# Asherchi/Stereo_Match_Traditional

Measured on AMD Instinct MI355X. Metric: Mdisparities/s (HxWxD/s) + ms/pair, AD-Census 1920x1080 D=192, higher is better.
Workload: dtype f32; 1 GPU; AD-Census 9x7 both views + WTA, 1920x1080 D=192 (adcensus_1080p_d192); parallelism=pairs sharded over 1 GPU(s), backend=none (single process), ranks_joined=1, ranks_joined_how=all_reduce(SUM) of 1 per rank over the job's communicator, world_size=1, launcher=none

## Files before the change

### stereo_match_traditional_amd/csrc/adcensus.hip

```cpp
#include "smt_common.h"
#include "adcensus_internal.h"
#include <math.h>
#include <stdlib.h>
#include <string.h>
#include <algorithm>
#include <new>
#include <type_traits>

namespace {

constexpr int TJ = 64;
constexpr int NT = 256;

struct Tables {
    uint64_t *cenA[2];
    uint64_t *cenX[2];
    uint64_t *mask;
    uint8_t *u8[2];
    float *lut;
    uint16_t *rank;
    int *flag;
    int WX;
    int edge_col;
    unsigned long long *stamp;
// ... 296 lines not shown
    }
}

#ifndef SMT_SHARED_KNOCKOUT
#define SMT_SHARED_KNOCKOUT 0
#endif
constexpr int SH_RING = 512;
constexpr int SH_RING_N = SH_RING + 4;
constexpr unsigned long long SH_NOKEY = ~0ull;
__host__ __device__ inline int shared_id_hi(int W, int D) { return W - 3 - D; }
__host__ __device__ inline int shared_pub_hi(int W) { return W - 4; }
__host__ __device__ inline bool shared_in_set(int c, int hi) { return (unsigned)(c - 3) <= (unsigned)(hi - 3) && hi >= 3; }
__host__ __device__ inline bool shared_publishes(int j, int c, int W, int pubhi) { return j <= W - 4 && shared_in_set(c, pubhi); }
__host__ __device__ inline unsigned long long shared_key(unsigned cost_bits, int d) { return ((unsigned long long)cost_bits << 32) | (unsigned)d; }
__host__ __device__ inline int shared_ring_base(int t, int C) { return (int)((unsigned)(t - (C - 1)) & (unsigned)(SH_RING - 1)); }
constexpr int SH_SPILL = SH_RING_N - SH_RING;
__host__ __device__ constexpr bool shared_walk_groups(int C, int Dfull) { return C == 3 && Dfull == 192; }
__host__ __device__ constexpr bool shared_ring_grouped(int C, int Dfull) { return C == 3 && Dfull == 192; }
static_assert(!shared_ring_grouped(3, 192) || shared_walk_groups(3, 192), "");
__host__ __device__ inline int shared_ring_slot(int t0, int u, int k, int C) { return shared_ring_base(t0, C) + u + (C - 1 - k); }
__host__ __device__ constexpr int shared_ring_spill(int C, bool grouped) { return grouped ? 2 * (C - 1) : C - 1; }
static_assert(shared_ring_spill(3, true) <= SH_SPILL && shared_ring_spill(4, false) <= SH_SPILL, "");
constexpr int SH_RUN = 4;
__host__ __device__ inline int shared_wg_chunks(int nbx, int H, int K, long b, int &i, int &bx)
{
    const long nb = (long)nbx * H, per = (nb + 7) >> 3, cl = (b >> 3) * K;
    if (cl >= per) return 0;
    const long c = (b & 7) * per + cl;
    if (c >= nb) return 0;
    i = (int)(c / nbx);
    bx = (int)(c - (long)i * nbx);
    long n = per - cl < nb - c ? per - cl : nb - c;
    return (int)(n < K ? n : K);
}
__host__ __device__ inline int shared_run_len(int nbx, int bx, int left)
{
    const int n = nbx - bx < SH_RUN ? nbx - bx : SH_RUN;
    return n < left ? n : left;
}
__host__ __device__ inline void shared_run_flush_range(int S, int E, int D, int pubhi, int &lo, int &hi)
{
    lo = S - D + 1 < 3 ? 3 : S - D + 1; hi = E > pubhi ? pubhi : E;
}
__host__ __device__ inline bool shared_complete(int c, int S, int E, int D) { return c >= S && c + D - 1 <= E; }
__host__ __device__ inline bool shared_complete(int c, int S, int E, int D, int idhi) { return c <= idhi && shared_complete(c, S, E, D); }
__host__ __device__ inline void shared_edge_range(int c, int W, int D, int &lo, int &hi)
{
    lo = c >= 3 && W - 3 - c > 0 ? W - 3 - c : 0;
    hi = W + 3 - c < D - 1 ? W + 3 - c : D - 1;
}
constexpr int SH_CONV_PX = 16 * 256;
constexpr int SH_EDGE_PX = 4 * 256;
constexpr int SH_EDGE0_PX = 16 * 4;
__host__ __device__ inline int shared_conv_items(int H, int W) { return (int)(((long)H * W + SH_CONV_PX - 1) / SH_CONV_PX); }
__host__ __device__ inline int shared_edge_cols(int W, int D) { return W - 1 - shared_id_hi(W, D); }
__host__ __device__ inline int shared_edge_col_items(int H, int W, int D)
// ... 213 lines not shown
                        const unsigned long long b = __ballot(ml == m);
                        const int first = __builtin_ctzll(b);
                        int kk = C - 1;
#pragma unroll
                        for (int k = C - 2; k >= 0; k--)
                            if ((unsigned)__builtin_amdgcn_readlane((int)key[k], first) == m) kk = k;
                        const int wd = first * C + kk;
                        res = (lane == q) ? wd : res;
                    }
                    const int ns = (VIEW == 0) ? (u + 1) % C : u % C;
                    rc[ns] = nc; rv[ns] = nv;
                }
            }
            anc_a += 16u * C; val_a += 2u * C;
            nx_a += 8u * C; nv_a += 2u * C;
        }
    };
    if (interior) run(std::false_type{});
    else run(std::true_type{});
    const int jw = j0 + p0 + lane;
    if (disp && lane < npx) disp[(size_t)i * W + jw] = (float)res;
}

__host__ __device__ inline bool chunk_decode(int nbx, int H, int nviews, int K, long b, int t, int &view, int &i, int &bx)
{
    const long nb = (long)nbx * H * nviews;
    const long per = (nb + 7) >> 3;
    const long cl = (b >> 3) * K + t;
    if (cl >= per) return false;
    const long c = (b & 7) * per + cl;
    if (c >= nb) return false;
    const long rows = (long)nbx * H;
    view = (int)(c / rows);
    const long r = c - (long)view * rows;
    i = (int)(r / nbx);
    bx = (int)(r - (long)i * nbx);
    return true;
}
__host__ __device__ inline int maps_groups(int nbx, int H, int nviews, int K)
{
    const long per = ((long)nbx * H * nviews + 7) >> 3;
    return (int)(8 * ((per + K - 1) / K));
}
__device__ __forceinline__ bool chunk_of_block(int nbx, int H, int nviews, int &view, int &i, int &bx, long b = -1)
{
    const long nb = (long)nbx * H * nviews;
    const long per = (nb + 7) >> 3;
    if (b < 0) b = blockIdx.x;
    const long c = (b & 7) * per + (b >> 3);
    if (c >= nb) return false;
    const long rows = (long)nbx * H;
    view = (int)(c / rows);
    const long r = c - (long)view * rows;
    i = (int)(r / nbx);
    bx = (int)(r - (long)i * nbx);
    return true;
}

template <int C, int VIEW, bool FULL>
__global__ void __launch_bounds__(NT) k_cost_fast(int H, int W, int D, Tables T, float *__restrict__ vol,
                                                  float *__restrict__ disp, int nbx)
{
    int view, i, bx;
    if (!chunk_of_block(nbx, H, 1, view, i, bx)) return;
    cost_fast_body<C, VIEW, FULL>(H, W, D, T, vol, disp, i, bx);
}

template <int C, bool FULL, bool NTS = true>
__global__ void __launch_bounds__(NT) k_cost_fast2(int H, int W, int D, Tables T, float *__restrict__ vol0,
                                                   float *__restrict__ vol1, float *__restrict__ disp0,
                                                   float *__restrict__ disp1, int nbx)
{
    int view, i, bx;
    if (!chunk_of_block(nbx, H, 2, view, i, bx)) return;
    unsigned long long t0 = 0, r0 = 0;
    if (T.stamp) { t0 = __builtin_amdgcn_s_memtime(); r0 = __builtin_amdgcn_s_memrealtime(); }
    if (view == 0) cost_fast_body<C, 0, FULL, NTS>(H, W, D, T, vol0, disp0, i, bx);
    else cost_fast_body<C, 1, FULL, NTS>(H, W, D, T, vol1, disp1, i, bx);
    if (T.stamp && threadIdx.x == 0) {
        unsigned long long *s = T.stamp + 4 * (size_t)blockIdx.x;
        s[0] = t0; s[1] = r0; s[2] = __builtin_amdgcn_s_memtime(); s[3] = __builtin_amdgcn_s_memrealtime();
    }
}

struct FusedGrid { int cgroups, pgroups, every, slots, groups; };
__host__ __device__ inline FusedGrid fused_grid(int ncost, int nprep)
{
    FusedGrid f;
    f.cgroups = ncost >> 3;
    f.pgroups = (nprep + 7) >> 3;
    f.every = f.cgroups / (f.pgroups > 0 ? f.pgroups : 1);
    if (f.every < 1) f.every = 1;
    f.slots = f.cgroups / f.every;
    f.groups = f.cgroups + (f.pgroups > f.slots ? f.pgroups : f.slots);
    return f;
}
__host__ __device__ inline bool fused_decode(const FusedGrid &f, int g, int &idx)
{
    const int period = f.every + 1, inter = f.slots * period;
    if (g < inter) {
        const int q = g / period, r = g - q * period;
        if (r == f.every) { idx = q; return true; }
        idx = q * f.every + r;
        return false;
    }
    const int g2 = g - inter, crest = f.cgroups - f.slots * f.every;
    if (g2 < crest) { idx = f.slots * f.every + g2; return false; }
    idx = f.slots + (g2 - crest);
    return true;
}

template <int C, bool FULL, bool NTS = true>
__global__ void __launch_bounds__(NT, 8) k_cost_fast2p(int H, int W, int D, Tables T, float *__restrict__ vol0,
// ... 57 lines not shown
            va = T.u8[view][(size_t)i * W + j];
        }
    }
    template <unsigned VSCALE, int TABN, int NBUF>
    __device__ __forceinline__ void store(MapsLds<C, TABN, NBUF> &ml, int buf, int Drt) const
    {
        const int D = FULL ? 64 * C : Drt, NX = FTJ + D, tid = threadIdx.x;
#pragma unroll
        for (int n = 0; n < NE; n++) {
            const int e = tid - (FULL ? 0 : XPAD) + n * NT;
            if (e < NX + (FULL ? 0 : XPAD)) {
                ml.st[buf].cenx[XPAD + e] = cen[n];
                ml.st[buf].valx[XPAD + e] = (uint16_t)(VSCALE * val[n]);
            }
        }
        if (tid < FTJ) { ml.st[buf].anc[tid] = anc; ml.st[buf].vala[tid] = (uint16_t)(VSCALE * va); }
    }
};

template <int C, bool FULL, int MODE>
__global__ void __launch_bounds__(NT) k_cost_maps2p(int H, int W, int D, Tables T, float *__restrict__ disp0,
                                                    float *__restrict__ disp1, int nbx, int K, int ncost, int nprep,
                                                    const float *__restrict__ nL, const float *__restrict__ nR,
                                                    Tables Tn, int ptx)
{
    static_assert(PNT == NT, "");
    constexpr int TABN = MapsCfg<MODE>::TABN, NBUF = MapsCfg<MODE>::NBUF;
    static_assert(2 * PSR * PSW * 4 <= TABN * 2 && 320 * 4 <= TABN * 2, "");
    __shared__ MapsLds<C, TABN, NBUF> lds;
    uint16_t *s_tab = lds.tab;
    long b = blockIdx.x;
    if (nprep > 0) {
        const FusedGrid f = fused_grid(ncost, nprep);
        int idx;
        const bool table = fused_decode(f, (int)(blockIdx.x >> 3), idx);
        b = idx * 8 + (int)(blockIdx.x & 7);
        if (table) {
            uint32_t (*sw)[PSW] = (uint32_t (*)[PSW])s_tab;
            if (b < nprep) prep_tile(nL, nR, H, W, Tn, (int)b % ptx, (int)b / ptx, ptx, sw, sw + PSR);
            return;
        }
    }
    const int tid = threadIdx.x;
    if (MODE == MODE_MAPS_RANK) {
        typedef unsigned u32x4 __attribute__((ext_vector_type(4)));
        for (int e = tid; e < RANK_N / 8; e += NT) ((u32x4 *)s_tab)[e] = ((const u32x4 *)T.rank)[e];
    } else {
        for (int e = tid; e < 320; e += NT) ((float *)s_tab)[e] = T.lut[e];
    }
    auto next = [&](int t, int &view, int &i, int &bx) {
        for (; t < K; t++) {
            if (!chunk_decode(nbx, H, 2, K, b, t, view, i, bx)) return K;
            if (view == 0 ? disp0 : disp1) return t;
        }
        return K;
    };
    MapsStage<C, FULL> st;
    int view = 0, i = 0, bx = 0;
    int t = next(0, view, i, bx);
    if (t < K) st.load(view, i, bx, W, D, T);
    bool first = true;
    int buf = 0;
    while (t < K) {
        if (NBUF == 1 && !first) __syncthreads();
        first = false;
        st.template store<MODE == MODE_MAPS_RANK ? 64u : 4u>(lds, buf, D);
        __syncthreads();
        const int cv = view, ci = i, cbx = bx;
        t = next(t + 1, view, i, bx);
        if (t < K) st.load(view, i, bx, W, D, T);
        if (cv == 0) cost_fast_body<C, 0, FULL, true, MODE>(H, W, D, T, nullptr, disp0, ci, cbx, &lds, buf);
        else cost_fast_body<C, 1, FULL, true, MODE>(H, W, D, T, nullptr, disp1, ci, cbx, &lds, buf);
        buf = NBUF == 1 ? 0 : buf ^ 1;
    }
}
// ... 276 lines not shown
        if (!shared_edge0_px(item - ncol, it, (int)(threadIdx.x >> 6), H, i, c)) return;
        const size_t p = (size_t)i * W + c;
        const uint64_t acen = T.cenA[1][p], amask = T.mask[p];
        const int va = T.u8[1][p];
        int lo, hi;
        shared_edge_range(c, W, D, lo, hi);
        unsigned long long k = SH_NOKEY;
        for (int d = lo + lane; d <= hi; d += 64) k = min(k, shared_edge_key(T, i, W, acen, amask, va, c + d, d));
#pragma unroll
        for (int s = 32; s >= 1; s >>= 1) k = min(k, (unsigned long long)__shfl_xor((long long)k, s));
        if (lane == 0) dispR[p] = (float)(unsigned)k;
    }
}

#ifndef SMT_SHARED_MIN_WAVES
#define SMT_SHARED_MIN_WAVES 7
#endif
template <int C, bool FULL>
__global__ void __launch_bounds__(NT, SMT_SHARED_MIN_WAVES) k_cost_maps_shared(int H, int W, int D, Tables T, float *__restrict__ disp0,
                                                         float *__restrict__ disp1, unsigned long long *__restrict__ keys,
                                                         int nbx, int K, int pubhi, int ncost, int nprep,
                                                         const float *__restrict__ nL, const float *__restrict__ nR,
                                                         Tables Tn, int ptx, int nconv, int nedge,
                                                         unsigned long long *__restrict__ ckeys, float *__restrict__ cdisp)
{
    static_assert(PNT == NT && NT == 256, "");
    static_assert(2 * PSR * PSW * 4 <= PREP_LDS_U16 * 2 && 320 * 4 <= PREP_LDS_U16 * 2, "");
    __shared__ RunLds<C> lds;
    __shared__ unsigned long long ring[SH_RING_N];
    long b;
    {
        const FusedGrid f = fused_grid(ncost, nprep + nconv + nedge);
        int idx;
        const bool table = fused_decode(f, (int)(blockIdx.x >> 3), idx);
        b = idx * 8 + (int)(blockIdx.x & 7);
        if (table) {
            int item;
            const int kind = shared_aux_decode((int)b, nprep, nconv, nedge, item);
            if (kind == AUX_PREP) {
                uint32_t (*sw)[PSW] = (uint32_t (*)[PSW])lds.tab;
                prep_tile(nL, nR, H, W, Tn, item % ptx, item / ptx, ptx, sw, sw + PSR);
            } else if (kind == AUX_CONV) shared_conv_item(ckeys, cdisp, (long)H * W, item);
            else if (kind == AUX_EDGE) shared_edge_item(T, H, W, FULL ? 64 * C : D, disp1, keys, item);
            return;
        }
    }
    const int tid = threadIdx.x;
    int i = 0, bx = 0;
    int left = shared_wg_chunks(nbx, H, K, b, i, bx);
    if (left == 0) return;
    for (int e = tid; e < 320; e += NT) ((float *)lds.tab)[e] = T.lut[e];
    const int Dd = FULL ? 64 * C : D;
    const int idhi = shared_id_hi(W, Dd);
    for (int e = tid; e < SH_RING_N; e += NT) ring[e] = SH_NOKEY;
    RunStage<C, FULL> st;
    int n = shared_run_len(nbx, bx, left);
    st.load(i, FTJ * bx, n, W, D, T);
    for (;;) {
        st.store(lds, n, D);
        __syncthreads();
        const int ci = i, cS = FTJ * bx, cn = n;
        left -= n; bx += n;
        if (bx == nbx) { bx = 0; i++; }
        n = shared_run_len(nbx, bx, left);
        shared_run_walk<C, FULL>(H, W, D, disp0, ci, cS, cn, &lds, ring, pubhi);
        if (n > 0) st.load(i, FTJ * bx, n, W, D, T);
        __syncthreads();
        const int cE = cS + FTJ * cn - 1;
        int lo, hi;
        shared_run_flush_range(cS, cE, Dd, pubhi, lo, hi);
        shared_flush<C, shared_ring_grouped(C, FULL ? 64 * C : 0)>(ring, ci, W, Dd, lo, hi, cS, cE, idhi, disp1, keys);
        if (n <= 0) break;
// ... 64 lines not shown
    hipStream_t stream;
    float *vol[2];
    Tables T;
    Tables TS[2];
    hipStream_t prep_stream;
    hipEvent_t in_ready, prep_done[2], cost_done[2];
    long n_pairs;
    hipEvent_t *ev;
    bool timing;
    bool force_generic;
    long n_timed;
    long n_seen;
    int timing_stride;
    bool *ev_merged;
    bool plain_stores;
    float store_mode_ms[2];
    int place_tries;
    float place_ms;
    unsigned long long *skeys[2];
    bool conv_pending;
    int conv_map;
    float *conv_dR;
    bool vol_lent, vol_pending;
};

SMT_API const char *smt_strerror(int s)
{
    switch (s) {
    case SMT_OK: return "ok";
    case SMT_ERR_ARG: return "invalid argument";
    case SMT_ERR_HIP: return "HIP runtime error";
    case SMT_ERR_ALLOC: return "device allocation failed";
    case SMT_ERR_DOMAIN: return "image values outside the integer 0..255 domain";
    case SMT_ERR_REF_UB: return "reference behaviour undefined for these inputs";
    case SMT_ERR_STATE: return "call order violated";
    default: return "unknown status";
    }
}
SMT_API int smt_version(void) { return SMT_VERSION; }
SMT_API int smt_last_hip_error(void) { return g_smt_last_hip; }
SMT_API int smt_device_count(int *n)
{
    if (!n) return SMT_ERR_ARG;
    SMT_HIP(hipGetDeviceCount(n));
    return SMT_OK;
}
// ... 169 lines not shown
            memcpy(&bits, &f, 4);
            kv[a * 64 + c] = ((uint64_t)bits << 32) | (uint32_t)(a * 64 + c);
        }
    std::sort(kv, kv + RANK_N);
    int r = -1;
    uint32_t prev = 0;
    for (int n = 0; n < RANK_N; n++) {
        const uint32_t bits = (uint32_t)(kv[n] >> 32);
        if (n == 0 || bits != prev) r++;
        prev = bits;
        rank[(uint32_t)kv[n]] = (uint16_t)r;
    }
    delete[] kv;
    return true;
}

static void flush_conversion(smt_adcensus *h)
{
    if (!h->conv_pending) return;
    const long N = (long)h->H * h->W;
    hipLaunchKernelGGL(k_shared_convert, dim3((unsigned)shared_conv_items(h->H, h->W)), dim3(NT), 0, h->stream,
                       h->skeys[h->conv_map], h->conv_dR, N);
    h->conv_pending = false;
}

static int adcensus_create(int H, int W, int D, float sigmaC, float sigmaS, unsigned flags, smt_adcensus **out)
{
    if (!out || H <= 0 || W <= 0 || D <= 0 || D > SMT_MAX_DISPARITY || !(sigmaC > 0.0f) || !(sigmaS > 0.0f) ||
        (long long)H * W >= (1ll << 31))
        return SMT_ERR_ARG;
    smt_adcensus *h = new (std::nothrow) smt_adcensus();
    if (!h) return SMT_ERR_ALLOC;
    h->device = smt_current_device();
    h->H = H; h->W = W; h->D = D; h->sigmaC = sigmaC; h->sigmaS = sigmaS;
    h->stream = nullptr; h->timing = false; h->force_generic = false; h->ev = nullptr; h->n_timed = 0; h->n_seen = 0; h->timing_stride = 1; h->ev_merged = nullptr;
    h->n_pairs = 0;
    const size_t N = (size_t)H * W, V = N * D;
    const int WX = W + 4;
    int rc = place_volumes(h, !(flags & SMT_ADCENSUS_NO_PLACEMENT_SEARCH));
    auto alloc = [&](void **p, size_t bytes) { if (rc == SMT_OK) rc = smt_malloc(p, bytes); };
    alloc((void **)&h->TS[0].lut, 320 * 4);
    alloc((void **)&h->TS[0].rank, RANK_N * 2);
    alloc((void **)&h->TS[0].flag, 4);
    for (int t = 0; t < 2; t++) {
        h->TS[t].WX = WX;
        h->TS[t].stamp = nullptr;
// ... 15 lines not shown
        smt_adcensus_destroy(h);
        return SMT_ERR_HIP;
    }
    for (int t = 0; t < 2; t++)
        if (hipEventCreateWithFlags(&h->prep_done[t], hipEventDisableTiming) != hipSuccess ||
            hipEventCreateWithFlags(&h->cost_done[t], hipEventDisableTiming) != hipSuccess) {
            smt_adcensus_destroy(h);
            return SMT_ERR_HIP;
        }
    float lut[320];
    build_lut(sigmaC, sigmaS, lut);
    uint16_t *rank = new (std::nothrow) uint16_t[RANK_N];
    if (!rank || !build_rank(lut, rank)) { delete[] rank; smt_adcensus_destroy(h); return SMT_ERR_ALLOC; }
    const bool rank_ok = hipMemcpy(h->TS[0].rank, rank, RANK_N * 2, hipMemcpyHostToDevice) == hipSuccess;
    delete[] rank;
    if (!rank_ok || hipMemcpy(h->TS[0].lut, lut, sizeof(lut), hipMemcpyHostToDevice) != hipSuccess ||
        hipMemset(h->vol[0], 0, V * 4) != hipSuccess || hipMemset(h->vol[1], 0, V * 4) != hipSuccess ||
        hipMemset(h->TS[0].flag, 0, 4) != hipSuccess || hipMemset(h->skeys[0], 0xFF, N * 8) != hipSuccess ||
        hipMemset(h->skeys[1], 0xFF, N * 8) != hipSuccess) {
        smt_adcensus_destroy(h);
        return SMT_ERR_HIP;
    }
    calibrate_store_mode(h, !(flags & SMT_ADCENSUS_NO_STORE_CALIBRATION));
    *out = h;
    return SMT_OK;
}

SMT_API int smt_adcensus_create(int H, int W, int D, float sigmaC, float sigmaS, smt_adcensus **out)
{
    return adcensus_create(H, W, D, sigmaC, sigmaS, 0u, out);
}

SMT_API int smt_adcensus_create_ex(int device, int H, int W, int D, float sigmaC, float sigmaS, unsigned flags, smt_adcensus **out)
{
    if (flags & ~(unsigned)(SMT_ADCENSUS_NO_PLACEMENT_SEARCH | SMT_ADCENSUS_NO_STORE_CALIBRATION)) return SMT_ERR_ARG;
    if (device < 0) return adcensus_create(H, W, D, sigmaC, sigmaS, flags, out);
    int n = 0;
    if (hipGetDeviceCount(&n) != hipSuccess || device >= n) return SMT_ERR_ARG;
    smt_dev_guard dev_guard(device);
    return adcensus_create(H, W, D, sigmaC, sigmaS, flags, out);
}

SMT_API int smt_adcensus_create_on(int device, int H, int W, int D, float sigmaC, float sigmaS, smt_adcensus **out)
{
    int n = 0;
    if (hipGetDeviceCount(&n) != hipSuccess || device < 0 || device >= n) return SMT_ERR_ARG;
// ... 45 lines not shown
    h->T.edge_col = h->TS[0].edge_col = h->TS[1].edge_col = col;
    return SMT_OK;
}

template <int C, bool FULL>
static void launch_cost(smt_adcensus *h, int view0, int nviews, float *d0, float *d1)
{
    const int D = h->D;
    dim3 grid((h->W + TJ - 1) / TJ, h->H, nviews);
    const int NX = TJ + D;
    size_t shm = (size_t)NX * 8 + TJ * 16 + 320 * 4 + NX + TJ;
    shm = (shm + 15) & ~(size_t)15;
    hipLaunchKernelGGL((k_cost<C, FULL>), grid, dim3(NT), shm, h->stream, h->H, h->W, D, h->T,
                       view0, h->vol[0], h->vol[1], d0, d1);
}

static int maps_chunks()
{
    const char *env = getenv("SMT_MAPS_CHUNKS");
    const int k = env ? atoi(env) : 0;
    return k >= 1 && k <= 64 ? k : 4;
}

static bool maps_shared()
{
    const char *env = getenv("SMT_MAPS_SHARED");
    return !(env && env[0] == '0' && env[1] == 0);
}
static bool maps_shared_shape(int W, int D)
{
    if (shared_id_hi(W, D) < 3) return false;
    const char *env = getenv("SMT_MAPS_SHARED");
    return D <= 192 || (env && env[0] == 'f');
}

static bool shared_finish_apart()
{
    const char *env = getenv("SMT_SHARED_FINISH");
    return env && strcmp(env, "apart") == 0;
}

static bool pair_takes_shared(const smt_adcensus *h, int views, const float *dL, const float *dR, bool maps)
{
    if (!(views == SMT_VIEW_BOTH && maps) || h->force_generic || (h->D + 63) / 64 > 4) return false;
    const char *env = getenv("SMT_MAPS_KERNEL");
    return !(env && env[0] == 'r') && dL && dR && maps_shared_shape(h->W, h->D) && maps_shared();
}

static int prep_items(int H, int W, int &ptx)
{
    ptx = (W + PTW - 1) / PTW;
    const int pty = (H + PTH - 1) / PTH, eb = (H + PNT / 16 - 1) / (PNT / 16);
    return ptx * (pty + (eb + ptx - 1) / ptx);
}

template <int C, bool FULL>
static void launch_fast(smt_adcensus *h, int views, float *dL, float *dR, const float *nL, const float *nR, bool maps)
{
    const int nbx = (h->W + FTJ - 1) / FTJ;
    auto blocks = [&](int nviews) { return dim3((unsigned)(((long)nbx * h->H * nviews + 7) / 8 * 8)); };
    if (views == SMT_VIEW_BOTH && maps) {
        const int K = maps_chunks();
        const int ncost = maps_groups(nbx, h->H, 2, K);
        int nprep = 0, ptx = 1;
        unsigned grid = (unsigned)ncost;
        if (nL) {
            nprep = prep_items(h->H, h->W, ptx);
            grid = 8u * (unsigned)fused_grid(ncost, nprep).groups;
        }
        const Tables &Tn = h->TS[(h->n_pairs + 1) & 1];
        const char *env = getenv("SMT_MAPS_KERNEL");
        if (pair_takes_shared(h, views, dL, dR, maps)) {
            const int km = (int)(h->n_pairs & 1);
            if (h->conv_pending && h->conv_map == km) flush_conversion(h);
            const bool carried = h->conv_pending;
            const int ncs = maps_groups(nbx, h->H, 1, K), Dd = FULL ? 64 * C : h->D;
            const int nconv = carried ? shared_conv_items(h->H, h->W) : 0, nedge = shared_edge_items(h->H, h->W, Dd);
            const unsigned gs = 8u * (unsigned)fused_grid(ncs, nprep + nconv + nedge).groups;
            hipLaunchKernelGGL((k_cost_maps_shared<C, FULL>), dim3(gs), dim3(NT), 0, h->stream, h->H, h->W, h->D, h->T, dL, dR,
                               h->skeys[km], nbx, K, shared_pub_hi(h->W), ncs, nprep, nL, nR, Tn, ptx, nconv, nedge,
                               carried ? h->skeys[h->conv_map] : nullptr, carried ? h->conv_dR : nullptr);
            if (SMT_SHARED_KNOCKOUT != 2) { h->conv_pending = true; h->conv_map = km; h->conv_dR = dR; }
            else h->conv_pending = false;
            if (shared_finish_apart()) flush_conversion(h);
            return;
        }
        if (env && env[0] == 'r')
            hipLaunchKernelGGL((k_cost_maps2p<C, FULL, MODE_MAPS_RANK>), dim3(grid), dim3(NT), 0, h->stream, h->H, h->W,
                               h->D, h->T, dL, dR, nbx, K, ncost, nprep, nL, nR, Tn, ptx);
        else
            hipLaunchKernelGGL((k_cost_maps2p<C, FULL, MODE_MAPS_FLOAT>), dim3(grid), dim3(NT), 0, h->stream, h->H, h->W,
                               h->D, h->T, dL, dR, nbx, K, ncost, nprep, nL, nR, Tn, ptx);
        return;
    }
    if (views == SMT_VIEW_BOTH && nL) {
        const int ncost = (int)blocks(2).x;
        const int ptx = (h->W + PTW - 1) / PTW, pty = (h->H + PTH - 1) / PTH;
        const int eb = (h->H + PNT / 16 - 1) / (PNT / 16);
        const int nprep = ptx * (pty + (eb + ptx - 1) / ptx);
        const unsigned grid = 8u * (unsigned)fused_grid(ncost, nprep).groups;
        const Tables &Tn = h->TS[(h->n_pairs + 1) & 1];
        if (h->plain_stores)
            hipLaunchKernelGGL((k_cost_fast2p<C, FULL, false>), dim3(grid), dim3(NT), 0, h->stream, h->H, h->W, h->D, h->T,
                               h->vol[0], h->vol[1], dL, dR, nbx, ncost, nprep, nL, nR, Tn, ptx);
        else
            hipLaunchKernelGGL((k_cost_fast2p<C, FULL, true>), dim3(grid), dim3(NT), 0, h->stream, h->H, h->W, h->D, h->T,
                               h->vol[0], h->vol[1], dL, dR, nbx, ncost, nprep, nL, nR, Tn, ptx);
        return;
    }
    if (views == SMT_VIEW_BOTH) {
        if (h->plain_stores)
            hipLaunchKernelGGL((k_cost_fast2<C, FULL, false>), blocks(2), dim3(NT), 0, h->stream, h->H, h->W, h->D, h->T, h->vol[0],
                               h->vol[1], dL, dR, nbx);
        else
            hipLaunchKernelGGL((k_cost_fast2<C, FULL, true>), blocks(2), dim3(NT), 0, h->stream, h->H, h->W, h->D, h->T, h->vol[0],
// ... 235 lines not shown
    const int pubhi = shared_pub_hi(W);
    const bool grouped = shared_ring_grouped(C, D == 64 * C ? D : 0);
    const size_t N = (size_t)H * W;
    static const float pal[] = {0.0f, 0.0f, 0.25f, 0.25f, 1.5f, 0.7265625f, 0.7265625f, 1.9999999f, 0.25f, 1e-30f};
    auto hash_bits = [&](int i, int j, int d, unsigned salt) {
        uint32_t x = (uint32_t)i * 0x9E3779B1u ^ (uint32_t)j * 0x85EBCA77u ^ (uint32_t)d * 0xC2B2AE3Du ^ seed * 0x27D4EB2Fu ^ salt;
        x ^= x >> 15; x *= 0x2C1B3C6Du; x ^= x >> 12; x *= 0x297A2D39u; x ^= x >> 15;
        float f = seed % 3 == 1 ? 0.5f : (seed % 3 == 2 && (x & 3)) ? (float)(x >> 12) * (1.0f / 1048576.0f) : pal[(x >> 4) % 10];
        uint32_t bits;
        memcpy(&bits, &f, 4);
        return bits;
    };
    auto cost_bits = [&](int i, int j, int d) { return hash_bits(i, j, d, 0u); };
    auto right_bits = [&](int i, int c, int d) {
        if (c >= 3 && c + d <= W - 4) return cost_bits(i, c + d, d);
        return hash_bits(i, c, std::min(d, W + 3 - c), 0x5BD1E995u);
    };
    unsigned long long *keys = new (std::nothrow) unsigned long long[N];
    unsigned *val = new (std::nothrow) unsigned[N]();
    unsigned char *nw = new (std::nothrow) unsigned char[N]();
    int rc = (keys && val && nw) ? SMT_OK : SMT_ERR_ALLOC;
    for (size_t p = 0; rc == SMT_OK && p < N; p++) keys[p] = SH_NOKEY;
    if (rc == SMT_OK && idhi >= 3) {
        const int nleft = maps_groups(nbx, H, 1, K);
        unsigned long long ring[SH_RING_N];
        int owner[SH_RING_N];
        for (long b = 0; b < nleft && rc == SMT_OK; b++) {
            for (int e = 0; e < SH_RING_N; e++) ring[e] = SH_NOKEY;
            int view, i, bx, ni, nbxn;
            int left = shared_wg_chunks(nbx, H, K, b, i, bx);
            for (int t = 0; t < K; t++)
                if (chunk_decode(nbx, H, 1, K, b, t, view, ni, nbxn) != (t < left)) rc = SMT_ERR_STATE;
            for (int t = 0; left > 0 && rc == SMT_OK;) {
                const int n = shared_run_len(nbx, bx, left);
                if (n < 1 || n > SH_RUN) { rc = SMT_ERR_STATE; break; }
                for (int u = 0; u < n; u++)
                    if (!chunk_decode(nbx, H, 1, K, b, t + u, view, ni, nbxn) || ni != i || nbxn != bx + u) rc = SMT_ERR_STATE;
                const int S = 64 * bx, E = S + 64 * n - 1;
                for (int e = 0; e < SH_RING_N; e++) owner[e] = -1;
                for (int j = S; j <= E && j < W; j++)
                    for (int lane = 0; lane < 64; lane++)
                        for (int k = 0; k < C; k++) {
                            const int dl = lane * C, d = dl + k, tcol = j - dl;
                            if (d >= D || !shared_publishes(j, tcol - k, W, pubhi)) continue;
                            const int u = grouped ? ((j - S) % (FPW * n)) % C : 0;
                            const int s = shared_ring_slot(tcol - u, u, k, C);
                            if (s < 0 || s >= SH_RING_N) { rc = SMT_ERR_STATE; continue; }
                            if (owner[s] != -1 && owner[s] != tcol - k) rc = SMT_ERR_STATE;
                            owner[s] = tcol - k;
                            ring[s] = std::min(ring[s], shared_key(cost_bits(i, j, d), d));
                        }
                int lo, hi;
                shared_run_flush_range(S, E, D, pubhi, lo, hi);
                for (int c = lo; c <= hi; c++) {
                    const int s = c & (SH_RING - 1);
                    unsigned long long k = ring[s];
                    ring[s] = SH_NOKEY;
                    if (s < shared_ring_spill(C, grouped)) { k = std::min(k, ring[SH_RING + s]); ring[SH_RING + s] = SH_NOKEY; }
                    const size_t p = (size_t)i * W + c;
                    if (shared_complete(c, S, E, D, idhi)) {
// ... 77 lines not shown
        for (size_t p = 0; p < N && rc == SMT_OK; p++)
            if (val2[p] != val[p] || nw2[p] != nw[p] || keys2[p] != keys[p]) rc = SMT_ERR_STATE;
        delete[] keys2; delete[] val2; delete[] nw2;
    }
    for (int i = 0; i < H && rc == SMT_OK; i++)
        for (int c = 0; c < W && rc == SMT_OK; c++) {
            const size_t p = (size_t)i * W + c;
            if (idhi < 3) { if (nw[p]) rc = SMT_ERR_STATE; continue; }
            if (keys[p] != SH_NOKEY) rc = SMT_ERR_STATE;
            float mn = 0.0f;
            int want = 0;
            for (int d = 0; d < D; d++) {
                const uint32_t bits = right_bits(i, c, d);
                float f;
                memcpy(&f, &bits, 4);
                if (d == 0 || f < mn) { mn = f; want = d; }
            }
            if (nw[p] != 1 || val[p] != (unsigned)want) rc = SMT_ERR_STATE;
        }
    delete[] keys; delete[] val; delete[] nw;
    return rc;
}

SMT_API int smt_adcensus_selftest_shared_aux_grid(int ncost, int nprep, int nedge, int nconv)
{
    if (ncost <= 0 || (ncost & 7) || nprep < 0 || nedge < 0 || nconv < 0) return SMT_ERR_ARG;
    const int naux = nprep + nconv + nedge;
    const FusedGrid f = fused_grid(ncost, naux);
    if (8L * f.groups < (long)ncost + naux) return SMT_ERR_STATE;
    unsigned char *cost = new (std::nothrow) unsigned char[(size_t)ncost]();
    unsigned char *aux = new (std::nothrow) unsigned char[(size_t)naux + 1]();
    int rc = (cost && aux) ? SMT_OK : SMT_ERR_ALLOC;
    for (long blk = 0; blk < 8L * f.groups && rc == SMT_OK; blk++) {
        int idx = -1;
        const bool table = fused_decode(f, (int)(blk >> 3), idx);
        if (idx < 0) { rc = SMT_ERR_STATE; break; }
        const long b = (long)idx * 8 + (blk & 7);
        if (!table) {
            if (b >= ncost || cost[b]++) rc = SMT_ERR_STATE;
            continue;
        }
        int item = -1;
        const int kind = shared_aux_decode((int)b, nprep, nconv, nedge, item);
        if (kind == AUX_NONE) { if (b < naux) rc = SMT_ERR_STATE; continue; }
        const int n = kind == AUX_PREP ? nprep : kind == AUX_CONV ? nconv : nedge;
        const int base = kind == AUX_PREP ? 0 : kind == AUX_CONV ? nprep : nprep + nconv;
        if (item < 0 || item >= n || base + item != b || aux[b]++) rc = SMT_ERR_STATE;
    }
    for (int c = 0; c < ncost && rc == SMT_OK; c++) if (cost[c] != 1) rc = SMT_ERR_STATE;
    for (int a = 0; a < naux && rc == SMT_OK; a++) if (aux[a] != 1) rc = SMT_ERR_STATE;
    delete[] cost; delete[] aux;
    return rc;
}

SMT_API int smt_adcensus_selftest_shared_aux(int H, int W, int D, int K, int first, int last)
{
    if (H <= 0 || W <= 0 || D <= 0 || D > 256 || K < 1 || K > 64 || (long)H * W > (1L << 24)) return SMT_ERR_ARG;
    const int idhi = shared_id_hi(W, D), nbx = (W + FTJ - 1) / FTJ;
    if (idhi < 3) return SMT_ERR_ARG;
    int ptx;
    const int ncost = maps_groups(nbx, H, 1, K), nprep = last ? 0 : prep_items(H, W, ptx);
    const int nconv = first ? 0 : shared_conv_items(H, W), nedge = shared_edge_items(H, W, D);
    int rc = smt_adcensus_selftest_shared_aux_grid(ncost, nprep, nedge, nconv);
    if (rc != SMT_OK) return rc;
    const long N = (long)H * W;
    unsigned char *seen = new (std::nothrow) unsigned char[(size_t)N]();
    if (!seen) return SMT_ERR_ALLOC;
    for (int item = 0; item < shared_conv_items(H, W); item++)
        for (int it = 0; it < SH_CONV_PX / 512; it++)
            for (int tid = 0; tid < 256; tid++) {
                long p;
                long p0;
                (void)shared_conv_px(item, 0, tid, N, p0);
                const bool in = shared_conv_px(item, it, tid, N, p);
                if (p != p0 + 512L * it) rc = SMT_ERR_STATE;
                if (!in) continue;
                if (p < 0 || (p & 1)) { rc = SMT_ERR_STATE; continue; }
                for (long e = p; e < p + 2 && e < N; e++) if (seen[e]++) rc = SMT_ERR_STATE;
            }
    for (long p = 0; p < N; p++) { if (seen[p] != 1) rc = SMT_ERR_STATE; seen[p] = 0; }
    const int ncol = shared_edge_col_items(H, W, D);
    for (int item = 0; item < nedge; item++)
        for (int it = 0; it < (item < ncol ? SH_EDGE_PX / 256 : SH_EDGE0_PX / 4); it++)
            for (int t = 0; t < (item < ncol ? 256 : 4); t++) {
                int i = -1, c = -1;
                if (!(item < ncol ? shared_edge_px(item, it, t, H, W, D, i, c) : shared_edge0_px(item - ncol, it, t, H, i, c)))
                    continue;
                const bool in = i >= 0 && i < H && (item < ncol ? c > idhi && c < W : c >= 0 && c < 3);
                if (!in || seen[(long)i * W + c]++) rc = SMT_ERR_STATE;
            }
    for (int i = 0; i < H; i++)
        for (int c = 0; c < W; c++) {
            const bool edge = c < 3 || c > idhi;
            if (seen[(long)i * W + c] != (edge ? 1 : 0)) rc = SMT_ERR_STATE;
            int lo, hi;
            shared_edge_range(c, W, D, lo, hi);
            if (c > idhi && c <= W - 4 && (lo > hi || lo < 1 || c + lo != W - 3)) rc = SMT_ERR_STATE;
            if (edge && (lo < 0 || hi > D - 1 || lo > hi)) rc = SMT_ERR_STATE;
        }
    delete[] seen;
    return rc;
}

SMT_API int smt_adcensus_selftest_cost_rank(float sigmaC, float sigmaS)
{
    if (!(sigmaC > 0.0f) || !(sigmaS > 0.0f)) return SMT_ERR_ARG;
    float lut[320];
    build_lut(sigmaC, sigmaS, lut);
    uint16_t *rank = new (std::nothrow) uint16_t[RANK_N];
    float *sum = new (std::nothrow) float[RANK_N];
    float *uniq = new (std::nothrow) float[RANK_N];
    int rc = (rank && sum && uniq && build_rank(lut, rank)) ? SMT_OK : SMT_ERR_ALLOC;
    int nu = 0;
    if (rc == SMT_OK) {
        for (int e = 0; e < RANK_N; e++) {
            sum[e] = lut[e >> 6] + lut[256 + (e & 63)];
            uint32_t bits;
            memcpy(&bits, &sum[e], 4);
            if (!(sum[e] >= 0.0f && sum[e] < INFINITY) || (bits >> 31)) rc = SMT_ERR_STATE;
            uniq[e] = sum[e];
        }
        std::sort(uniq, uniq + RANK_N);
        nu = (int)(std::unique(uniq, uniq + RANK_N) - uniq);
    }
    for (int e = 0; e < RANK_N && rc == SMT_OK; e++) {
        const int below = (int)(std::lower_bound(uniq, uniq + nu, sum[e]) - uniq);
// ... 180 lines not shown
```

### stereo_match_traditional_amd/csrc/adcensus_internal.h

```cpp
#pragma once
#include "smt_common.h"

int adcensus_batch_pairs(smt_adcensus *h, const float *L, const float *R, int n, int views, float *dispL,
                         float *dispR, int sched, bool prepped, const float *nL, const float *nR, bool maps_ok,
                         bool last_volumes);
bool adcensus_fused_both_views(const smt_adcensus *h);
SMT_API int smt_adcensus_selftest_shared_keys(int H, int W, int D, int K, unsigned seed);
SMT_API int smt_adcensus_selftest_shared_aux_grid(int ncost, int nprep, int nedge, int nconv);
SMT_API int smt_adcensus_selftest_shared_aux(int H, int W, int D, int K, int first, int last);
```

Baseline: 1.984 million Mdisp/s.

## Taper chunk spans at grid tail to balance the maps kernel's last wave

Workgroups normally process K chunks each. This change lets the final groups take half-K or single-chunk spans, so the tail of the grid finishes more evenly. The tail sizes come from occupancy-derived resident-block counts that are queried at create time. By default n1 is set to one resident wave of single-chunk groups whenever the grid exceeds one wave. Fused aux/prep groups are interleaved only inside the body, so tail groups hold pure cost work. The cost is more groups with per-group table-load overhead and more decode logic.

After: 2.029 million Mdisp/s (median of 6 runs). 1.02x the previous value.

```diff
diff --git a/stereo_match_traditional_amd/csrc/adcensus.hip b/stereo_match_traditional_amd/csrc/adcensus.hip
--- a/stereo_match_traditional_amd/csrc/adcensus.hip
+++ b/stereo_match_traditional_amd/csrc/adcensus.hip
@@ -342,16 +342,49 @@
 __host__ __device__ constexpr int shared_ring_spill(int C, bool grouped) { return grouped ? 2 * (C - 1) : C - 1; }
 static_assert(shared_ring_spill(3, true) <= SH_SPILL && shared_ring_spill(4, false) <= SH_SPILL, "");
 constexpr int SH_RUN = 4;
-__host__ __device__ inline int shared_wg_chunks(int nbx, int H, int K, long b, int &i, int &bx)
-{
-    const long nb = (long)nbx * H, per = (nb + 7) >> 3, cl = (b >> 3) * K;
-    if (cl >= per) return 0;
+__host__ __device__ inline long maps_span_tails(long per, int K, int &n2, int &n1)
+{
+    const int K2 = K > 1 ? K >> 1 : 1;
+    if (n1 < 0) n1 = 0;
+    if (n2 < 0) n2 = 0;
+    if (n1 > per) n1 = (int)per;
+    const long rem = per - n1;
+    if ((long)n2 * K2 > rem) n2 = (int)(rem / K2);
+    return rem - (long)n2 * K2;
+}
+__host__ __device__ inline int maps_span(long per, int K, int n2, int n1, long g, long &first)
+{
+    const long body = maps_span_tails(per, K, n2, n1);
+    first = g * K;
+    if (first < body) return (int)(body - first < K ? body - first : K);
+    const int K2 = K > 1 ? K >> 1 : 1;
+    const long gt = g - (body + K - 1) / K;
+    if (gt < n2) { first = body + gt * K2; return K2; }
+    first = body + (long)n2 * K2 + (gt - n2);
+    return gt - n2 < n1 ? 1 : 0;
+}
+__host__ __device__ inline long maps_span_body(long per, int K, int n2, int n1)
+{
+    return (maps_span_tails(per, K, n2, n1) + K - 1) / K;
+}
+__host__ __device__ inline long maps_span_groups(long per, int K, int n2, int n1)
+{
+    const long nbody = maps_span_body(per, K, n2, n1);
+    (void)maps_span_tails(per, K, n2, n1);
+    return nbody + n2 + n1;
+}
+__host__ __device__ inline int shared_wg_chunks(int nbx, int H, int K, long b, int &i, int &bx, int n2 = 0, int n1 = 0)
+{
+    const long nb = (long)nbx * H, per = (nb + 7) >> 3;
+    long cl;
+    const int m = maps_span(per, K, n2, n1, b >> 3, cl);
+    if (m <= 0) return 0;
     const long c = (b & 7) * per + cl;
     if (c >= nb) return 0;
     i = (int)(c / nbx);
     bx = (int)(c - (long)i * nbx);
-    long n = per - cl < nb - c ? per - cl : nb - c;
-    return (int)(n < K ? n : K);
+    const long n = nb - c;
+    return (int)(n < m ? n : m);
 }
 __host__ __device__ inline int shared_run_len(int nbx, int bx, int left)
 {
@@ -611,12 +644,10 @@
     if (disp && lane < npx) disp[(size_t)i * W + jw] = (float)res;
 }
 
-__host__ __device__ inline bool chunk_decode(int nbx, int H, int nviews, int K, long b, int t, int &view, int &i, int &bx)
+__host__ __device__ inline bool chunk_at(int nbx, int H, int nviews, long b, long cl, int &view, int &i, int &bx)
 {
     const long nb = (long)nbx * H * nviews;
     const long per = (nb + 7) >> 3;
-    const long cl = (b >> 3) * K + t;
-    if (cl >= per) return false;
     const long c = (b & 7) * per + cl;
     if (c >= nb) return false;
     const long rows = (long)nbx * H;
@@ -626,10 +657,24 @@
     bx = (int)(r - (long)i * nbx);
     return true;
 }
-__host__ __device__ inline int maps_groups(int nbx, int H, int nviews, int K)
+__host__ __device__ inline bool chunk_decode(int nbx, int H, int nviews, int K, long b, int t, int &view, int &i, int &bx,
+                                             int n2 = 0, int n1 = 0)
 {
     const long per = ((long)nbx * H * nviews + 7) >> 3;
-    return (int)(8 * ((per + K - 1) / K));
+    long first;
+    if (t >= maps_span(per, K, n2, n1, b >> 3, first)) return false;
+    return chunk_at(nbx, H, nviews, b, first + t, view, i, bx);
+}
+__host__ __device__ inline int maps_groups(int nbx, int H, int nviews, int K, int n2 = 0, int n1 = 0)
+{
+    const long per = ((long)nbx * H * nviews + 7) >> 3;
+    return (int)(8 * maps_span_groups(per, K, n2, n1));
+}
+__host__ __device__ inline int maps_body_groups(int nbx, int H, int nviews, int K, int n2, int n1)
+{
+    const long per = ((long)nbx * H * nviews + 7) >> 3;
+    (void)maps_span_tails(per, K, n2, n1);
+    return n2 + n1 > 0 ? (int)maps_span_body(per, K, n2, n1) : 0;
 }
 __device__ __forceinline__ bool chunk_of_block(int nbx, int H, int nviews, int &view, int &i, int &bx, long b = -1)
 {
@@ -673,11 +718,17 @@
 }
 
 struct FusedGrid { int cgroups, pgroups, every, slots, groups; };
-__host__ __device__ inline FusedGrid fused_grid(int ncost, int nprep)
+__host__ __device__ inline FusedGrid fused_grid(int ncost, int nprep, int cbody = 0)
 {
     FusedGrid f;
     f.cgroups = ncost >> 3;
     f.pgroups = (nprep + 7) >> 3;
+    if (cbody > 0 && f.pgroups > 0 && cbody >= f.pgroups && cbody < f.cgroups) {
+        f.every = cbody / f.pgroups;
+        f.slots = f.pgroups;
+        f.groups = f.cgroups + f.pgroups;
+        return f;
+    }
     f.every = f.cgroups / (f.pgroups > 0 ? f.pgroups : 1);
     if (f.every < 1) f.every = 1;
     f.slots = f.cgroups / f.every;
@@ -781,7 +832,7 @@
 __global__ void __launch_bounds__(NT) k_cost_maps2p(int H, int W, int D, Tables T, float *__restrict__ disp0,
                                                     float *__restrict__ disp1, int nbx, int K, int ncost, int nprep,
                                                     const float *__restrict__ nL, const float *__restrict__ nR,
-                                                    Tables Tn, int ptx)
+                                                    Tables Tn, int ptx, int n2, int n1, int cbody)
 {
     static_assert(PNT == NT, "");
     constexpr int TABN = MapsCfg<MODE>::TABN, NBUF = MapsCfg<MODE>::NBUF;
@@ -790,7 +841,7 @@
     uint16_t *s_tab = lds.tab;
     long b = blockIdx.x;
     if (nprep > 0) {
-        const FusedGrid f = fused_grid(ncost, nprep);
+        const FusedGrid f = fused_grid(ncost, nprep, cbody);
         int idx;
         const bool table = fused_decode(f, (int)(blockIdx.x >> 3), idx);
         b = idx * 8 + (int)(blockIdx.x & 7);
@@ -807,9 +858,11 @@
     } else {
         for (int e = tid; e < 320; e += NT) ((float *)s_tab)[e] = T.lut[e];
     }
+    long c0;
+    const int m = maps_span((((long)nbx * H * 2) + 7) >> 3, K, n2, n1, b >> 3, c0);
     auto next = [&](int t, int &view, int &i, int &bx) {
-        for (; t < K; t++) {
-            if (!chunk_decode(nbx, H, 2, K, b, t, view, i, bx)) return K;
+        for (; t < m; t++) {
+            if (!chunk_at(nbx, H, 2, b, c0 + t, view, i, bx)) return K;
             if (view == 0 ? disp0 : disp1) return t;
         }
         return K;
@@ -1132,7 +1185,8 @@
                                                          int nbx, int K, int pubhi, int ncost, int nprep,
                                                          const float *__restrict__ nL, const float *__restrict__ nR,
                                                          Tables Tn, int ptx, int nconv, int nedge,
-                                                         unsigned long long *__restrict__ ckeys, float *__restrict__ cdisp)
+                                                         unsigned long long *__restrict__ ckeys, float *__restrict__ cdisp,
+                                                         int n2, int n1, int cbody)
 {
     static_assert(PNT == NT && NT == 256, "");
     static_assert(2 * PSR * PSW * 4 <= PREP_LDS_U16 * 2 && 320 * 4 <= PREP_LDS_U16 * 2, "");
@@ -1140,7 +1194,7 @@
     __shared__ unsigned long long ring[SH_RING_N];
     long b;
     {
-        const FusedGrid f = fused_grid(ncost, nprep + nconv + nedge);
+        const FusedGrid f = fused_grid(ncost, nprep + nconv + nedge, cbody);
         int idx;
         const bool table = fused_decode(f, (int)(blockIdx.x >> 3), idx);
         b = idx * 8 + (int)(blockIdx.x & 7);
@@ -1157,7 +1211,7 @@
     }
     const int tid = threadIdx.x;
     int i = 0, bx = 0;
-    int left = shared_wg_chunks(nbx, H, K, b, i, bx);
+    int left = shared_wg_chunks(nbx, H, K, b, i, bx, n2, n1);
     if (left == 0) return;
     for (int e = tid; e < 320; e += NT) ((float *)lds.tab)[e] = T.lut[e];
     const int Dd = FULL ? 64 * C : D;
@@ -1268,6 +1322,7 @@
     int conv_map;
     float *conv_dR;
     bool vol_lent, vol_pending;
+    int maps_resident[3];
 };
 
 SMT_API const char *smt_strerror(int s)
@@ -1483,6 +1538,34 @@
     hipLaunchKernelGGL(k_shared_convert, dim3((unsigned)shared_conv_items(h->H, h->W)), dim3(NT), 0, h->stream,
                        h->skeys[h->conv_map], h->conv_dR, N);
     h->conv_pending = false;
+}
+
+template <int C, bool FULL>
+static void query_maps_resident(smt_adcensus *h, int cus)
+{
+    int n[3] = {0, 0, 0};
+    if (hipOccupancyMaxActiveBlocksPerMultiprocessor(&n[0], k_cost_maps_shared<C, FULL>, NT, 0) != hipSuccess) n[0] = 0;
+    if (hipOccupancyMaxActiveBlocksPerMultiprocessor(&n[1], k_cost_maps2p<C, FULL, MODE_MAPS_FLOAT>, NT, 0) != hipSuccess) n[1] = 0;
+    if (hipOccupancyMaxActiveBlocksPerMultiprocessor(&n[2], k_cost_maps2p<C, FULL, MODE_MAPS_RANK>, NT, 0) != hipSuccess) n[2] = 0;
+    for (int t = 0; t < 3; t++) h->maps_resident[t] = n[t] > 0 ? cus / 8 * n[t] : 0;
+}
+static void set_maps_resident(smt_adcensus *h)
+{
+    h->maps_resident[0] = h->maps_resident[1] = h->maps_resident[2] = 0;
+    int cus = 0;
+    if (hipDeviceGetAttribute(&cus, hipDeviceAttributeMultiprocessorCount, h->device) != hipSuccess || cus < 8) return;
+    switch ((h->D + 63) / 64 * 2 + (h->D % 64 == 0 ? 1 : 0)) {
+    case 3: query_maps_resident<1, true>(h, cus); break;
+    case 5: query_maps_resident<2, true>(h, cus); break;
+    case 7: query_maps_resident<3, true>(h, cus); break;
+    case 9: query_maps_resident<4, true>(h, cus); break;
+    case 2: query_maps_resident<1, false>(h, cus); break;
+    case 4: query_maps_resident<2, false>(h, cus); break;
+    case 6: query_maps_resident<3, false>(h, cus); break;
+    case 8: query_maps_resident<4, false>(h, cus); break;
+    default: break;
+    }
+    (void)hipGetLastError();
 }
 
 static int adcensus_create(int H, int W, int D, float sigmaC, float sigmaS, unsigned flags, smt_adcensus **out)
@@ -1544,6 +1627,7 @@
         return SMT_ERR_HIP;
     }
     calibrate_store_mode(h, !(flags & SMT_ADCENSUS_NO_STORE_CALIBRATION));
+    set_maps_resident(h);
     *out = h;
     return SMT_OK;
 }
@@ -1635,6 +1719,21 @@
     return k >= 1 && k <= 64 ? k : 4;
 }
 
+constexpr int TAPER_N2_HALVES = 0, TAPER_N1_HALVES = 2;
+static void maps_taper(int S, long per, int K, int &n2, int &n1)
+{
+    n2 = n1 = 0;
+    const char *env = getenv("SMT_MAPS_TAPER");
+    if (env && env[0]) {
+        int a = 0, b = 0;
+        if (sscanf(env, "%d,%d", &a, &b) == 2 && a >= 0 && b >= 0) { n2 = a; n1 = b; }
+    } else if (S > 0 && maps_span_groups(per, K, 0, 0) > S) {
+        n2 = (int)((long)S * TAPER_N2_HALVES / 2);
+        n1 = (int)((long)S * TAPER_N1_HALVES / 2);
+    }
+    (void)maps_span_tails(per, K, n2, n1);
+}
+
 static bool maps_shared()
 {
     const char *env = getenv("SMT_MAPS_SHARED");
@@ -1674,36 +1773,38 @@
     auto blocks = [&](int nviews) { return dim3((unsigned)(((long)nbx * h->H * nviews + 7) / 8 * 8)); };
     if (views == SMT_VIEW_BOTH && maps) {
         const int K = maps_chunks();
-        const int ncost = maps_groups(nbx, h->H, 2, K);
         int nprep = 0, ptx = 1;
-        unsigned grid = (unsigned)ncost;
-        if (nL) {
-            nprep = prep_items(h->H, h->W, ptx);
-            grid = 8u * (unsigned)fused_grid(ncost, nprep).groups;
-        }
+        if (nL) nprep = prep_items(h->H, h->W, ptx);
         const Tables &Tn = h->TS[(h->n_pairs + 1) & 1];
         const char *env = getenv("SMT_MAPS_KERNEL");
+        int n2, n1;
         if (pair_takes_shared(h, views, dL, dR, maps)) {
             const int km = (int)(h->n_pairs & 1);
             if (h->conv_pending && h->conv_map == km) flush_conversion(h);
             const bool carried = h->conv_pending;
-            const int ncs = maps_groups(nbx, h->H, 1, K), Dd = FULL ? 64 * C : h->D;
+            maps_taper(h->maps_resident[0], ((long)nbx * h->H + 7) >> 3, K, n2, n1);
+            const int ncs = maps_groups(nbx, h->H, 1, K, n2, n1), Dd = FULL ? 64 * C : h->D;
+            const int cbody = maps_body_groups(nbx, h->H, 1, K, n2, n1);
             const int nconv = carried ? shared_conv_items(h->H, h->W) : 0, nedge = shared_edge_items(h->H, h->W, Dd);
-            const unsigned gs = 8u * (unsigned)fused_grid(ncs, nprep + nconv + nedge).groups;
+            const unsigned gs = 8u * (unsigned)fused_grid(ncs, nprep + nconv + nedge, cbody).groups;
             hipLaunchKernelGGL((k_cost_maps_shared<C, FULL>), dim3(gs), dim3(NT), 0, h->stream, h->H, h->W, h->D, h->T, dL, dR,
                                h->skeys[km], nbx, K, shared_pub_hi(h->W), ncs, nprep, nL, nR, Tn, ptx, nconv, nedge,
-                               carried ? h->skeys[h->conv_map] : nullptr, carried ? h->conv_dR : nullptr);
+                               carried ? h->skeys[h->conv_map] : nullptr, carried ? h->conv_dR : nullptr, n2, n1, cbody);
             if (SMT_SHARED_KNOCKOUT != 2) { h->conv_pending = true; h->conv_map = km; h->conv_dR = dR; }
             else h->conv_pending = false;
             if (shared_finish_apart()) flush_conversion(h);
             return;
         }
-        if (env && env[0] == 'r')
+        const bool rank = env && env[0] == 'r';
+        maps_taper(h->maps_resident[rank ? 2 : 1], ((long)nbx * h->H * 2 + 7) >> 3, K, n2, n1);
+        const int ncost = maps_groups(nbx, h->H, 2, K, n2, n1), cbody = maps_body_groups(nbx, h->H, 2, K, n2, n1);
+        const unsigned grid = nL ? 8u * (unsigned)fused_grid(ncost, nprep, cbody).groups : (unsigned)ncost;
+        if (rank)
             hipLaunchKernelGGL((k_cost_maps2p<C, FULL, MODE_MAPS_RANK>), dim3(grid), dim3(NT), 0, h->stream, h->H, h->W,
-                               h->D, h->T, dL, dR, nbx, K, ncost, nprep, nL, nR, Tn, ptx);
+                               h->D, h->T, dL, dR, nbx, K, ncost, nprep, nL, nR, Tn, ptx, n2, n1, cbody);
         else
             hipLaunchKernelGGL((k_cost_maps2p<C, FULL, MODE_MAPS_FLOAT>), dim3(grid), dim3(NT), 0, h->stream, h->H, h->W,
-                               h->D, h->T, dL, dR, nbx, K, ncost, nprep, nL, nR, Tn, ptx);
+                               h->D, h->T, dL, dR, nbx, K, ncost, nprep, nL, nR, Tn, ptx, n2, n1, cbody);
         return;
     }
     if (views == SMT_VIEW_BOTH && nL) {
@@ -1985,20 +2086,22 @@
     int rc = (keys && val && nw) ? SMT_OK : SMT_ERR_ALLOC;
     for (size_t p = 0; rc == SMT_OK && p < N; p++) keys[p] = SH_NOKEY;
     if (rc == SMT_OK && idhi >= 3) {
-        const int nleft = maps_groups(nbx, H, 1, K);
+        int n2, n1;
+        maps_taper(0, ((long)nbx * H + 7) >> 3, K, n2, n1);
+        const int nleft = maps_groups(nbx, H, 1, K, n2, n1);
         unsigned long long ring[SH_RING_N];
         int owner[SH_RING_N];
         for (long b = 0; b < nleft && rc == SMT_OK; b++) {
             for (int e = 0; e < SH_RING_N; e++) ring[e] = SH_NOKEY;
             int view, i, bx, ni, nbxn;
-            int left = shared_wg_chunks(nbx, H, K, b, i, bx);
+            int left = shared_wg_chunks(nbx, H, K, b, i, bx, n2, n1);
             for (int t = 0; t < K; t++)
-                if (chunk_decode(nbx, H, 1, K, b, t, view, ni, nbxn) != (t < left)) rc = SMT_ERR_STATE;
+                if (chunk_decode(nbx, H, 1, K, b, t, view, ni, nbxn, n2, n1) != (t < left)) rc = SMT_ERR_STATE;
             for (int t = 0; left > 0 && rc == SMT_OK;) {
                 const int n = shared_run_len(nbx, bx, left);
                 if (n < 1 || n > SH_RUN) { rc = SMT_ERR_STATE; break; }
                 for (int u = 0; u < n; u++)
-                    if (!chunk_decode(nbx, H, 1, K, b, t + u, view, ni, nbxn) || ni != i || nbxn != bx + u) rc = SMT_ERR_STATE;
+                    if (!chunk_decode(nbx, H, 1, K, b, t + u, view, ni, nbxn, n2, n1) || ni != i || nbxn != bx + u) rc = SMT_ERR_STATE;
                 const int S = 64 * bx, E = S + 64 * n - 1;
                 for (int e = 0; e < SH_RING_N; e++) owner[e] = -1;
                 for (int j = S; j <= E && j < W; j++)
@@ -2122,15 +2225,18 @@
     return rc;
 }
 
-SMT_API int smt_adcensus_selftest_shared_aux_grid(int ncost, int nprep, int nedge, int nconv)
-{
-    if (ncost <= 0 || (ncost & 7) || nprep < 0 || nedge < 0 || nconv < 0) return SMT_ERR_ARG;
+static int shared_aux_grid_check(int ncost, int nprep, int nedge, int nconv, int cbody)
+{
+    if (ncost <= 0 || (ncost & 7) || nprep < 0 || nedge < 0 || nconv < 0 || cbody < 0) return SMT_ERR_ARG;
     const int naux = nprep + nconv + nedge;
-    const FusedGrid f = fused_grid(ncost, naux);
+    const FusedGrid f = fused_grid(ncost, naux, cbody), f0 = fused_grid(ncost, naux);
     if (8L * f.groups < (long)ncost + naux) return SMT_ERR_STATE;
+    if (cbody == 0 && (f.every != f0.every || f.slots != f0.slots || f.groups != f0.groups)) return SMT_ERR_STATE;
+    const bool in_body = cbody > 0 && cbody < f.cgroups && f.pgroups > 0 && cbody >= f.pgroups;
     unsigned char *cost = new (std::nothrow) unsigned char[(size_t)ncost]();
     unsigned char *aux = new (std::nothrow) unsigned char[(size_t)naux + 1]();
     int rc = (cost && aux) ? SMT_OK : SMT_ERR_ALLOC;
+    bool tapered = false;
     for (long blk = 0; blk < 8L * f.groups && rc == SMT_OK; blk++) {
         int idx = -1;
         const bool table = fused_decode(f, (int)(blk >> 3), idx);
@@ -2138,8 +2244,10 @@
         const long b = (long)idx * 8 + (blk & 7);
         if (!table) {
             if (b >= ncost || cost[b]++) rc = SMT_ERR_STATE;
+            if (in_body && idx >= cbody) tapered = true;
             continue;
         }
+        if (in_body && tapered) rc = SMT_ERR_STATE;
         int item = -1;
         const int kind = shared_aux_decode((int)b, nprep, nconv, nedge, item);
         if (kind == AUX_NONE) { if (b < naux) rc = SMT_ERR_STATE; continue; }
@@ -2152,6 +2260,10 @@
     delete[] cost; delete[] aux;
     return rc;
 }
+SMT_API int smt_adcensus_selftest_shared_aux_grid(int ncost, int nprep, int nedge, int nconv)
+{
+    return shared_aux_grid_check(ncost, nprep, nedge, nconv, 0);
+}
 
 SMT_API int smt_adcensus_selftest_shared_aux(int H, int W, int D, int K, int first, int last)
 {
@@ -2159,9 +2271,11 @@
     const int idhi = shared_id_hi(W, D), nbx = (W + FTJ - 1) / FTJ;
     if (idhi < 3) return SMT_ERR_ARG;
     int ptx;
-    const int ncost = maps_groups(nbx, H, 1, K), nprep = last ? 0 : prep_items(H, W, ptx);
+    int n2, n1;
+    maps_taper(0, ((long)nbx * H + 7) >> 3, K, n2, n1);
+    const int ncost = maps_groups(nbx, H, 1, K, n2, n1), nprep = last ? 0 : prep_items(H, W, ptx);
     const int nconv = first ? 0 : shared_conv_items(H, W), nedge = shared_edge_items(H, W, D);
-    int rc = smt_adcensus_selftest_shared_aux_grid(ncost, nprep, nedge, nconv);
+    int rc = shared_aux_grid_check(ncost, nprep, nedge, nconv, maps_body_groups(nbx, H, 1, K, n2, n1));
     if (rc != SMT_OK) return rc;
     const long N = (long)H * W;
     unsigned char *seen = new (std::nothrow) unsigned char[(size_t)N]();
@@ -2202,6 +2316,46 @@
     return rc;
 }
 
+SMT_API int smt_adcensus_selftest_spans(long nb, int K, int n2, int n1)
+{
+    if (nb <= 0 || nb > (1L << 28) || K < 1 || K > 64 || n2 < 0 || n1 < 0) return SMT_ERR_ARG;
+    const long per = (nb + 7) >> 3, ng = maps_span_groups(per, K, n2, n1);
+    unsigned char *seen = new (std::nothrow) unsigned char[(size_t)nb]();
+    if (!seen) return SMT_ERR_ALLOC;
+    int rc = SMT_OK, e2 = n2, e1 = n1;
+    const long body = maps_span_tails(per, K, e2, e1);
+    const int K2 = K > 1 ? K >> 1 : 1;
+    if (body < 0 || e2 > n2 || e1 > n1 || body + (long)e2 * K2 + e1 != per || ng != (body + K - 1) / K + e2 + e1) rc = SMT_ERR_STATE;
+    for (int x = 0; x < 8 && rc == SMT_OK; x++) {
+        long expect = 0;
+        for (long g = 0; g < ng + 2 && rc == SMT_OK; g++) {
+            long first = -1;
+            const int m = maps_span(per, K, n2, n1, g, first);
+            if (g >= ng) { if (m != 0) rc = SMT_ERR_STATE; continue; }
+            if (m < 1 || m > K || first != expect || first + m > per) { rc = SMT_ERR_STATE; break; }
+            if (g >= ng - e1 ? m != 1 : g >= ng - e1 - e2 ? m != K2 : (m != K && g != ng - e1 - e2 - 1)) rc = SMT_ERR_STATE;
+            if (n1 == 0 && n2 == 0) {
+                const long cl = g * K, lim = per - cl < K ? per - cl : K;
+                if (first != cl || m != lim) rc = SMT_ERR_STATE;
+            }
+            expect = first + m;
+            for (long c = x * per + first; c < x * per + first + m; c++)
+                if (c < nb && seen[c]++) rc = SMT_ERR_STATE;
+        }
+        if (expect != per) rc = SMT_ERR_STATE;
+    }
+    for (long c = 0; c < nb && rc == SMT_OK; c++) if (seen[c] != 1) rc = SMT_ERR_STATE;
+    for (long b = 0; b < 8 * ng && rc == SMT_OK && nb <= (1L << 20); b++) {
+        long first;
+        int i = -1, bx = -1;
+        const int m = maps_span(per, K, n2, n1, b >> 3, first), got = shared_wg_chunks(1, (int)nb, K, b, i, bx, n2, n1);
+        const long c = (b & 7) * per + first, want = c >= nb ? 0 : (nb - c < m ? nb - c : m);
+        if (got != want || (got > 0 && (i != c || bx != 0))) rc = SMT_ERR_STATE;
+    }
+    delete[] seen;
+    return rc;
+}
+
 SMT_API int smt_adcensus_selftest_cost_rank(float sigmaC, float sigmaS)
 {
     if (!(sigmaC > 0.0f) || !(sigmaS > 0.0f)) return SMT_ERR_ARG;
diff --git a/stereo_match_traditional_amd/csrc/adcensus_internal.h b/stereo_match_traditional_amd/csrc/adcensus_internal.h
--- a/stereo_match_traditional_amd/csrc/adcensus_internal.h
+++ b/stereo_match_traditional_amd/csrc/adcensus_internal.h
@@ -8,3 +8,4 @@
 SMT_API int smt_adcensus_selftest_shared_keys(int H, int W, int D, int K, unsigned seed);
 SMT_API int smt_adcensus_selftest_shared_aux_grid(int ncost, int nprep, int nedge, int nconv);
 SMT_API int smt_adcensus_selftest_shared_aux(int H, int W, int D, int K, int first, int last);
+SMT_API int smt_adcensus_selftest_spans(long nb, int K, int n2, int n1);
```
